# geduardo/SPARC

Measured on AMD Instinct MI355X. Metric: env-steps/sec at batch 65536, higher is better.
Workload: dtype f32 wire temperature + f64 scalar state

## Files before the change

### sparc_amd/csrc/wedm_common.h

```cpp
#pragma once


#ifndef WEDM_PACKED_DENSE
#define WEDM_PACKED_DENSE true
#endif
#ifndef WEDM_FUSED_DENSE
#define WEDM_FUSED_DENSE false
#endif
#ifndef WEDM_FUSED_MIN_BLOCKS
#define WEDM_FUSED_MIN_BLOCKS 2
#endif
#ifndef WEDM_PACKED_MIN_BLOCKS
#define WEDM_PACKED_MIN_BLOCKS 2
#endif
#ifndef WEDM_STREAM_PAIRED_LOADS
#define WEDM_STREAM_PAIRED_LOADS 1
#endif
#ifndef WEDM_STREAM_DENSE_QUIET
#define WEDM_STREAM_DENSE_QUIET 1
#endif
#ifndef WEDM_STREAM_REGWALK
#define WEDM_STREAM_REGWALK 1
#endif
#ifndef WEDM_PIN_STAGE
// ... 383 lines not shown
__device__ __forceinline__ void quad_f64(const f2 (&tm)[4], const f2 (&tc)[4], const f2 (&tp)[4], f2 (&tn)[4], const Geom& g,
                                         const f2 (&hc)[4], const Persist& ps, const f2 (&jfl)[4], const StencilF64& h, double jf64) {
    double cA = (double)hc[0].x * g.a64, cB = (double)hc[0].y * g.a64;
    double jA = (JOULE && jfl[0].x != 0.0f) ? jf64 : 0.0, jB = (JOULE && jfl[0].y != 0.0f) ? jf64 : 0.0;
#pragma unroll
    for (int u = 0; u < 4; ++u) {
        if (PERCELL && u > 0) {
            cA = (double)hc[u].x * g.a64; cB = (double)hc[u].y * g.a64;
            jA = (JOULE && jfl[u].x != 0.0f) ? jf64 : 0.0; jB = (JOULE && jfl[u].y != 0.0f) ? jf64 : 0.0;
        }
        tn[u].x = cell_f64<JOULE>(tm[u].x, tc[u].x, tp[u].x, g.k64, g.tuf64, cA, h.tdiel, ps.adv64, jA, h.alpha, h.tref);
#if WEDM_REGS_F64_FENCE < 0
        __builtin_amdgcn_sched_barrier(0);
#endif
        tn[u].y = cell_f64<JOULE>(tm[u].y, tc[u].y, tp[u].y, g.k64, g.tuf64, cB, h.tdiel, ps.adv64, jB, h.alpha, h.tref);
#if WEDM_REGS_F64_FENCE < 0
        __builtin_amdgcn_sched_barrier(0);
#elif WEDM_REGS_F64_FENCE > 0
        if ((u + 1) % WEDM_REGS_F64_FENCE == 0) __builtin_amdgcn_sched_barrier(0);
#endif
    }
}

template <bool F64, bool JOULE, bool PERCELL, int SW>
__device__ __forceinline__ void rw_quad(const f2 (&tm)[4], const f2 (&tc)[4], const f2 (&tp)[4], f2 (&tn)[4], const Geom& g,
                                        const f2 (&conv)[4], float tdiel, const Persist& ps, const f2 (&jfe)[4], float alpha,
                                        float tref, const StencilF64& h, const Coef& cf) {
    if (F64) quad_f64<JOULE, PERCELL>(tm, tc, tp, tn, g, conv, ps, jfe, h, cf.jf64);
    else quad_staged<JOULE, PERCELL, SW>(tm, tc, tp, tn, g.k, g.tuf, conv, tdiel, ps.adv, jfe, alpha, tref);
}
template <bool F64>
__device__ __forceinline__ float rw_cell(int i, int n_seg, float tm1, float tc, float tp1, const Geom& g, const Coef& cf,
                                         const Persist& ps, float tref, float alpha, float tdiel, const StencilF64& h,
                                         float h_base, float h_zone) {
    if (F64) return stencil_cell_f64(i, n_seg, tm1, tc, tp1, g, cf, ps, h, h_base, h_zone);
    return stencil_cell(i, n_seg, tm1, tc, tp1, g, cf, ps, tref, alpha, tdiel);
}

#define WEDM_REPORT_FROZEN(cond)                                                      \
    do {                                                                              \
        if (!kFrozenOk && __any(cond)) {                                              \
            int32_t* const seen = cold->frozen_seen;                                  \
            if (seen && (threadIdx.x & 63) == 0) *seen = 1;                           \
        }                                                                             \
    } while (0)

#ifdef WEDM_STAMPS
#define WEDM_STAMP(var)                                                      \
    do {                                                                     \
        __builtin_amdgcn_sched_barrier(0);                                   \
        asm volatile("s_memtime %0\n\ts_waitcnt lgkmcnt(0)" : "=s"(var)::"memory"); \
        __builtin_amdgcn_sched_barrier(0);                                   \
    } while (0)
#define WEDM_STAMP_DECL unsigned long long st0 = 0, st1 = 0, st2 = 0, st3 = 0, st4 = 0, acc0 = 0, acc1 = 0, acc2 = 0, acc3 = 0, tk0 = 0, tk1 = 0, accN = 0, accB = 0, accS = 0, cntN = 0, cntB = 0, cntS = 0
#define WEDM_STAMP_ACC() do { acc0 += st1 - st0; acc1 += st2 - st1; acc2 += st3 - st2; acc3 += st4 - st3; } while (0)
#define WEDM_STAMP_ACC_SPLIT(quiet)                                                             \
    do {                                                                                        \
        if (quiet) { WEDM_STAMP_ACC(); ++cntS; }                                                \
        else { accN += st1 - st0; accB += st2 - st1; accS += st4 - st2; ++cntN; }               \
    } while (0)
#define WEDM_STAMP_OUT()                                                                         \
    do {                                                                                         \
        if (k.dbg && (threadIdx.x & 63) == 0) {                                                  \
            unsigned long long* o = k.dbg + ((size_t)blockIdx.x * 4 + (threadIdx.x >> 6)) * 4;   \
            o[0] = acc0; o[1] = acc1; o[2] = acc2; o[3] = acc3;                                  \
            unsigned long long* o2 = k.dbg + (size_t)gridDim.x * 16 + ((size_t)blockIdx.x * 4 + (threadIdx.x >> 6)) * 6; \
            o2[0] = accN; o2[1] = accB; o2[2] = accS; o2[3] = cntN; o2[4] = cntB; o2[5] = cntS;  \
        }                                                                                        \
    } while (0)
#else
#define WEDM_STAMP(var) do { } while (0)
#define WEDM_STAMP_DECL do { } while (0)
#define WEDM_STAMP_ACC() do { } while (0)
#define WEDM_STAMP_ACC_SPLIT(quiet) do { } while (0)
#define WEDM_STAMP_OUT() do { } while (0)
#endif
```

### sparc_amd/csrc/wedm_device.h

```cpp
#pragma once

#include <hip/hip_runtime.h>
#include <stdint.h>

#include "../../include/wedm_hip.h"
#include "wedm_env_rows.h"

namespace wedm {

enum : uint32_t {
    F_TRACE = 1u << 0,
    F_F64 = 1u << 1,
    F_REPLAY = 1u << 2,
    F_PULSE = 1u << 3,
    F_ENVP = 1u << 4,
    F_MAT = 1u << 5,
    F_FROZEN_OK = 1u << 6,
    F_N1 = 1u << 7,
    F_EXTRA = 1u << 8,
    F_CUT = 1u << 9,
    F_ONE = 1u << 10,
    F_CMAX104 = 1u << 11,
    F_MINB2 = 1u << 12,
    F_SIG = 1u << 13,
// ... 92 lines not shown
struct W4 { uint32_t x, y, z, w; };

__device__ __forceinline__ W4 philox4(uint32_t key0, uint32_t key1, uint32_t time, uint32_t episode,
                                      uint32_t gid, uint32_t stream) {
    uint32_t c0 = time, c1 = episode, c2 = gid, c3 = stream, k0 = key0, k1 = key1;
#pragma unroll
    for (int r = 0; r < 10; ++r) {
        uint64_t p0 = (uint64_t)0xD2511F53u * c0;
        uint64_t p1 = (uint64_t)0xCD9E8D57u * c2;
        uint32_t n0 = (uint32_t)(p1 >> 32) ^ c1 ^ k0, n2 = (uint32_t)(p0 >> 32) ^ c3 ^ k1;
        c0 = n0; c1 = (uint32_t)p1; c2 = n2; c3 = (uint32_t)p0;
        k0 += 0x9E3779B9u;
        k1 += 0xBB67AE85u;
    }
    return W4{c0, c1, c2, c3};
}

__device__ __forceinline__ double u32_to_unit(uint32_t w) { return ((double)w + 0.5) * 2.3283064365386963e-10; }

struct U2 { double a, b; };
__device__ __forceinline__ U2 philox_pair(uint32_t key0, uint32_t key1, uint32_t time, uint32_t episode,
                                           uint32_t gid, uint32_t stream) {
    W4 w = philox4(key0, key1, time, episode, gid, stream);
    U2 u;
    u.a = ((double)(w.x >> 5) * 67108864.0 + (double)(w.y >> 6)) / 9007199254740992.0;
    u.b = ((double)(w.z >> 5) * 67108864.0 + (double)(w.w >> 6)) / 9007199254740992.0;
    return u;
}

__device__ __forceinline__ double philox_std_normal(uint32_t key0, uint32_t key1, uint32_t time,
                                                    uint32_t episode, uint32_t gid) {
    for (uint32_t j = 0; j < 64; ++j) {
        U2 u = philox_pair(key0, key1, time, episode, gid, 1u + j);
        double v1 = 2.0 * u.a - 1.0, v2 = 2.0 * u.b - 1.0;
        double s = v1 * v1 + v2 * v2;
        if (s < 1.0 && s != 0.0) return v1 * sqrt(-2.0 * portable_log(s) / s);
    }
    return 0.0;
}

struct Env {
    double wp, x, v, prev_a;
    double debris, rho, flow, last_gap, last_rho, wire_last_flow;
    double V, I, y, last_crater, cavity;
    double tdelta, tvolt, on, off, tpos, unwind;
    double ipk;
    double vacc;
    float h_base, h_zone, tmax;
    int32_t time, tss, tsov, tsi, tse, dur, rnd_rem, deb_rem, tcrit, mode, episode, sparks;
    uint32_t key0, key1;
    int32_t state;
    int32_t is_short, broken, reached, done, ctrl, err;
};

struct Hot {
    double hard_short_gap, base_critical_density, gap_coefficient, max_critical_density, sigmoid_steepness;
    double ignition_a, ignition_b, ignition_c, ln2;
    double default_target_voltage, default_on_time, default_off_time, spark_voltage_factor;
    double debris_removal_per_us;
    double dt_s, damping_coeff, stiffness_coeff, omega_n, max_acceleration, max_jerk_dt, max_speed;
    float spool, tref, alpha, tdiel, tcrit, tbreak;
    int32_t servo_interval, dt_us, control_mode, disable_ignition, has_random_short, per_env_geometry;
    uint32_t env_id_offset;
    int32_t n_seg;
    int32_t done_value;
};

__device__ __forceinline__ void pin_hot_in_vgprs(Hot& h) {
#define WEDM_PIN(x) asm volatile("" : "+v"(h.x))
    WEDM_PIN(hard_short_gap); WEDM_PIN(base_critical_density); WEDM_PIN(gap_coefficient);
    WEDM_PIN(max_critical_density); WEDM_PIN(sigmoid_steepness);
    WEDM_PIN(ignition_a); WEDM_PIN(ignition_b); WEDM_PIN(ignition_c); WEDM_PIN(ln2);
    WEDM_PIN(default_target_voltage); WEDM_PIN(default_on_time); WEDM_PIN(default_off_time);
    WEDM_PIN(spark_voltage_factor); WEDM_PIN(debris_removal_per_us);
    WEDM_PIN(dt_s); WEDM_PIN(damping_coeff); WEDM_PIN(stiffness_coeff); WEDM_PIN(omega_n);
    WEDM_PIN(max_acceleration); WEDM_PIN(max_jerk_dt); WEDM_PIN(max_speed);
#undef WEDM_PIN
}

__device__ __forceinline__ const double* kernarg_envp();
#define WEDM_ENVP_ROW(rows, row, stride) ((rows)[(int64_t)(row) * (stride) + e])

__device__ __forceinline__ void envp_apply(Hot& h, int64_t stride, int64_t e) {
    const double* const r = kernarg_envp();
    h.base_critical_density = WEDM_ENVP_ROW(r, WEDM_EP_BASE_CRITICAL_DENSITY, stride);
    h.gap_coefficient = WEDM_ENVP_ROW(r, WEDM_EP_GAP_COEFFICIENT, stride);
    h.max_critical_density = WEDM_ENVP_ROW(r, WEDM_EP_MAX_CRITICAL_DENSITY, stride);
    h.hard_short_gap = WEDM_ENVP_ROW(r, WEDM_EP_HARD_SHORT_GAP, stride);
    h.sigmoid_steepness = WEDM_ENVP_ROW(r, WEDM_EP_SIGMOID_STEEPNESS, stride);
    h.spark_voltage_factor = WEDM_ENVP_ROW(r, WEDM_EP_SPARK_VOLTAGE_FACTOR, stride);
    h.debris_removal_per_us = WEDM_ENVP_ROW(r, WEDM_EP_DEBRIS_REMOVAL_PER_US, stride);
    h.tdiel = (float)WEDM_ENVP_ROW(r, WEDM_EP_DIELECTRIC_TEMPERATURE, stride);
    h.damping_coeff = WEDM_ENVP_ROW(r, WEDM_EP_DAMPING_COEFF, stride);
    h.stiffness_coeff = WEDM_ENVP_ROW(r, WEDM_EP_STIFFNESS_COEFF, stride);
    h.omega_n = WEDM_ENVP_ROW(r, WEDM_EP_OMEGA_N, stride);
    h.max_acceleration = WEDM_ENVP_ROW(r, WEDM_EP_MAX_ACCELERATION, stride);
    h.max_jerk_dt = WEDM_ENVP_ROW(r, WEDM_EP_MAX_JERK_DT, stride);
    h.max_speed = WEDM_ENVP_ROW(r, WEDM_EP_MAX_SPEED, stride);
}

__device__ __forceinline__ const double* kernarg_wmat();
#define WEDM_WMAT_ROW(rows, row, stride) ((rows)[(int64_t)(row) * (stride) + e])

__device__ __forceinline__ void wmat_apply(Hot& h, int64_t stride, int64_t e) {
    const double* const r = kernarg_wmat();
    h.alpha = (float)WEDM_WMAT_ROW(r, WEDM_WM_ALPHA_RHO, stride);
// ... 582 lines not shown
        cf.jf = 0.0f;
        cf.jf64 = 0.0;
        if (cf.joule_on) {
            const double joule_geom = p.per_env_geometry ? cc0->g.f64[(int64_t)WEDM_G_JOULE_GEOM * cc0->s.stride + e] : jg_u;
            cf.jf64 = joule_geom * I2 * (MAT ? WEDM_WMAT_ROW(kernarg_wmat(), WEDM_WM_RHO_ELEC, cc0->s.stride) : rho_elec);
            cf.jf = (float)cf.jf64;
        }
    }
    return cf;
}

__device__ __forceinline__ bool pair_lane_b() { return (threadIdx.x & 1u) != 0u; }
__device__ __forceinline__ uint32_t pair_from_a(uint32_t x) { return (uint32_t)__builtin_amdgcn_mov_dpp((int32_t)x, 0xA0, 0xF, 0xF, true); }
__device__ __forceinline__ uint32_t pair_from_b(uint32_t x) { return (uint32_t)__builtin_amdgcn_mov_dpp((int32_t)x, 0xF5, 0xF, 0xF, true); }
__device__ __forceinline__ double pair_from_a(double x) {
    const uint64_t u = d2bits(x);
    return bits2d(((uint64_t)pair_from_a((uint32_t)(u >> 32)) << 32) | pair_from_a((uint32_t)u));
}
__device__ __forceinline__ double pair_from_b(double x) {
    const uint64_t u = d2bits(x);
    return bits2d(((uint64_t)pair_from_b((uint32_t)(u >> 32)) << 32) | pair_from_b((uint32_t)u));
}

#ifndef WEDM_PAIR_KEYS_HOISTED
#define WEDM_PAIR_KEYS_HOISTED 0
#endif
#ifndef WEDM_PAIR_DIV
#define WEDM_PAIR_DIV 1
#endif
struct PhiloxHalf { uint32_t X, lo; };
__device__ __forceinline__ PhiloxHalf philox4_pair(bool lane_b, uint32_t key0, uint32_t key1, uint32_t time, uint32_t episode,
                                                   uint32_t gid, uint32_t stream) {
#if !WEDM_PAIR_KEYS_HOISTED
    uint32_t odd = lane_b ? 1u : 0u;
    asm volatile("" : "+v"(odd));
    lane_b = odd != 0u;
#endif
    const uint32_t mul = lane_b ? 0xCD9E8D57u : 0xD2511F53u, weyl = lane_b ? 0xBB67AE85u : 0x9E3779B9u;
    uint32_t X = lane_b ? gid : time, lo = lane_b ? episode : stream, k = lane_b ? key1 : key0;
#pragma unroll
    for (int r = 0; r < 10; ++r) {
        const uint64_t m = (uint64_t)mul * X;
        const uint32_t t = (uint32_t)(m >> 32) ^ lo;
        lo = (uint32_t)m;
        X = (uint32_t)swap_with_neighbour((int32_t)t) ^ k;
        k += weyl;
    }
    return PhiloxHalf{X, lo};
}
__device__ __forceinline__ W4 philox4_pair_words(PhiloxHalf h) {
    return W4{pair_from_a(h.X), pair_from_b(h.lo), pair_from_b(h.X), pair_from_a(h.lo)};
}

template <bool DENSE, uint32_t F = 0, bool PAIR = false>
__device__ __forceinline__ bool quiet_prelude_t(const Hot& p, const ColdRef cold, const Geom& g, int64_t e, uint32_t gid,
                                                Env& s, QuietTry& qt, Coef& cf) {
    constexpr bool ENVP = (F & F_ENVP) != 0, MAT = (F & F_MAT) != 0;
    qt.have_w = false;
    if (p.disable_ignition || p.has_random_short) return false;
    const bool live = !s.done;
    const double d0 = s.wp - s.x;
    const bool idle = s.state == 0, rest = s.state == -2;
    const bool spk = DENSE && s.state == 1;
    double crit = p.base_critical_density + p.gap_coefficient * d0;
    crit = crit < p.max_critical_density ? crit : p.max_critical_density;
    const double ex = -p.sigmoid_steepness * (s.rho - crit);
    bool q = (s.tss < p.servo_interval) && (s.rnd_rem == 0) && (s.deb_rem == 0) && (idle || rest || spk) &&
             (d0 >= p.hard_short_gap) && (ex > 24.0);
    const double cavity = g.cavity_coeff * (d0 * 0.001);
    double rho = 0.0;
    double lam_pair = 0.0;
    if (PAIR && WEDM_PAIR_DIV) {
        const bool lane_b = pair_lane_b();
        const double den = p.ignition_a * (d0 * d0) + p.ignition_b * d0 + p.ignition_c;
        const double quot = (lane_b ? p.ln2 : s.debris) / (lane_b ? den : cavity);
        const double qq = pair_from_a(quot);
        lam_pair = pair_from_b(quot);
        if (cavity > 0) rho = qq < 1.0 ? qq : 1.0;
    } else if (cavity > 0) {
        const double qq = s.debris / cavity;
        rho = qq < 1.0 ? qq : 1.0;
    }
    q = q && !(__builtin_fabs(d0 - s.last_gap) > 0.01 || __builtin_fabs(rho - s.last_rho) > 0.001) &&
        !(__builtin_fabs(s.flow - s.wire_last_flow) > 0.01) && (d0 > 0.001);
    if (!__all(q || !live)) return false;
    bool ign = false;
    PhiloxHalf wh{0u, 0u};
    if (__any(idle && live)) {
        if (PAIR) {
            wh = philox4_pair(pair_lane_b(), s.key0, s.key1, (uint32_t)s.time, (uint32_t)s.episode, gid, 0u);
            if (!WEDM_PAIR_DIV) lam_pair = p.ln2 / (p.ignition_a * (d0 * d0) + p.ignition_b * d0 + p.ignition_c);
            ign = idle && live && (u32_to_unit(pair_from_b(wh.X)) < lam_pair);
        } else {
            const double lam = p.ln2 / (p.ignition_a * (d0 * d0) + p.ignition_b * d0 + p.ignition_c);
            const W4 w = philox4(s.key0, s.key1, (uint32_t)s.time, (uint32_t)s.episode, gid, 0u);
            ign = idle && live && (u32_to_unit(w.z) < lam);
#ifndef WEDM_NO_PHILOX_REUSE
            qt.w = w;
#endif
        }
#ifndef WEDM_NO_PHILOX_REUSE
        qt.have_w = true;
#endif
    }
    if (__any(ign)) {
#ifndef WEDM_NO_PHILOX_REUSE
        if (PAIR) qt.w = philox4_pair_words(wh);
#endif
        return false;
    }
    bool burning = false;
    if (live) {
        const double Vt = s.tvolt != 0.0 ? s.tvolt : p.default_target_voltage;
        const double on = s.on != 0.0 ? s.on : p.default_on_time;
        const double off = s.off != 0.0 ? s.off : p.default_off_time;
        const int32_t dur1 = s.dur + 1;
        const bool end_rest = rest && ((double)dur1 >= on + off);
        const bool end_on = spk && ((double)dur1 >= on);
        burning = spk && !end_on;
        s.ctrl = 0;
        s.is_short = 0;
        double V = idle ? Vt : (end_rest ? Vt : 0.0);
        if (DENSE) V = spk ? (end_on ? 0.0 : Vt * p.spark_voltage_factor) : V;
        s.V = V;
        s.I = burning ? s.ipk : 0.0;
        s.y = end_rest ? __builtin_nan("") : s.y;
        s.dur = idle ? s.dur : (end_rest ? 0 : dur1);
        s.state = end_rest ? 0 : (end_on ? -2 : s.state);
        s.last_crater = 0.0;
        s.cavity = cavity;
        s.rho = rho;
        if (s.flow > 0.001 && s.debris > 0.001) {
            const double nv = s.debris - p.debris_removal_per_us * s.flow;
            s.debris = nv > 0.0 ? nv : 0.0;
        }
    }
    if (DENSE && __any(burning)) {
        const ColdPtr cc0 = cold.get();
        const ParamsPtr c = opaque(cc0->p);
        const double seg = c->segment_len, eff = c->plasma_efficiency, rho_elec = c->rho_elec;
        const int zone_start = (p.per_env_geometry && burning) ? cc0->g.i32[(int64_t)WEDM_GI_ZONE_START * cc0->s.stride + e] : c->zone_start;
        const double joule_geom = (p.per_env_geometry && burning) ? cc0->g.f64[(int64_t)WEDM_G_JOULE_GEOM * cc0->s.stride + e] : c->joule_geom;
        if (burning && s.y == s.y) {
            const int idx = seg != 0 ? zone_start + spark_cell_offset(s.y, seg) : zone_start;
            if (idx >= 0 && idx < g.n_seg) {
                cf.pidx = idx;
                cf.q64 = (ENVP ? WEDM_ENVP_ROW(kernarg_envp(), WEDM_EP_PLASMA_EFFICIENCY, cc0->s.stride) : eff) * s.V * s.I;
                cf.q = (float)cf.q64;
            }
        }
        if (burning) {
            const double I2 = s.I * s.I;
            cf.joule_on = I2 > 1e-6;
            if (cf.joule_on) {
                cf.jf64 = joule_geom * I2 * (MAT ? WEDM_WMAT_ROW(kernarg_wmat(), WEDM_WM_RHO_ELEC, cc0->s.stride) : rho_elec);
                cf.jf = (float)cf.jf64;
            }
        }
    }
    return true;
}

__device__ __forceinline__ bool quiet_prelude(const Hot& p, const Geom& g, uint32_t gid, Env& s, QuietTry& qt) {
    Coef unused{0.0f, 0.0f, 0, -1};
    return quiet_prelude_t<false>(p, ColdRef{nullptr}, g, 0, gid, s, qt, unused);
}

__device__ __forceinline__ bool quiet_prelude(const Hot& p, const Geom& g, uint32_t gid, Env& s) {
    QuietTry qt;
    return quiet_prelude(p, g, gid, s, qt);
}

__device__ __forceinline__ float sub_twice(float a, float b) { return __builtin_fmaf(-2.0f, b, a); }
typedef float f2v __attribute__((ext_vector_type(2)));
__device__ __forceinline__ f2v sub_twice(f2v a, f2v b) {
    const f2v m2 = {-2.0f, -2.0f};
    return __builtin_elementwise_fma(m2, b, a);
}

__device__ __forceinline__ float stencil_cell(int i, int n_seg, float tm1, float tc, float tp1, const Geom& g,
                                              const Coef& c, const Persist& ps, float tref, float alpha,
                                              float tdiel) {
// ... 326 lines not shown
```

### sparc_amd/csrc/wedm_env_rows.h

```cpp
#pragma once

#define WEDM_ENV_F64_DOUBLES(X, a) \
    X(a, wp,             WEDM_F_WORKPIECE_POS,  PRE_GENERAL, IN,          STATE)  \
    X(a, x,              WEDM_F_WIRE_POS,       EPILOGUE,    IN,          STATE)  \
    X(a, v,              WEDM_F_WIRE_VEL,       EPILOGUE,    IN,          STATE)  \
    X(a, prev_a,         WEDM_F_PREV_ACCEL,     EPILOGUE,    IN,          MODULE) \
    X(a, debris,         WEDM_F_DEBRIS_VOLUME,  PRE_QUIET,   IN,          MODULE) \
    X(a, rho,            WEDM_F_DEBRIS_DENSITY, PRE_QUIET,   IN,          STATE)  \
    X(a, flow,           WEDM_F_FLOW,           PRE_GENERAL, IN,          MODULE) \
    X(a, last_gap,       WEDM_F_LAST_GAP,       PRE_GENERAL, IN,          MODULE) \
    X(a, last_rho,       WEDM_F_LAST_DENSITY,   PRE_GENERAL, IN,          MODULE) \
    X(a, wire_last_flow, WEDM_F_WIRE_LAST_FLOW, PRE_GENERAL, IN,          MODULE) \
    X(a, V,              WEDM_F_VOLTAGE,        PRE_QUIET,   IN,          STATE)  \
    X(a, I,              WEDM_F_CURRENT,        PRE_QUIET,   IN_FORCED,   STATE)  \
    X(a, y,              WEDM_F_SPARK_Y,        PRE_QUIET,   IN,          STATE)  \
    X(a, last_crater,    WEDM_F_LAST_CRATER,    PRE_QUIET,   OUT,         STATE)  \
    X(a, cavity,         WEDM_F_CAVITY,         PRE_QUIET,   OUT,         STATE)  \
    X(a, tdelta,         WEDM_F_TARGET_DELTA,   PRE_GENERAL, IN,          STATE)  \
    X(a, tvolt,          WEDM_F_TARGET_VOLTAGE, PRE_GENERAL, IN,          STATE)  \
    X(a, on,             WEDM_F_ON_TIME,        PRE_GENERAL, IN,          STATE)  \
    X(a, off,            WEDM_F_OFF_TIME,       PRE_GENERAL, IN,          STATE)  \
    X(a, tpos,           WEDM_F_TARGET_POS,     NEVER,       IN,          STATE)  \
    X(a, unwind,         WEDM_F_UNWIND_VEL,     NEVER,       IN,          STATE)
#define WEDM_ENV_F64_SUMS(X, a) \
    X(a, vacc,           WEDM_F_VOLT_ACC,       EPILOGUE,    IN,          STATE)
#define WEDM_ENV_F64_FLOATS(X, a) \
    X(a, h_base,         WEDM_F_H_BASE,         PRE_GENERAL, IN,          MODULE) \
    X(a, h_zone,         WEDM_F_H_ZONE,         PRE_GENERAL, IN,          MODULE) \
    X(a, tmax,           WEDM_F_TMAX,           EPILOGUE,    IN_KEEPSTEP, STATE)
#define WEDM_ENV_F64(X, a) WEDM_ENV_F64_DOUBLES(X, a) WEDM_ENV_F64_SUMS(X, a) WEDM_ENV_F64_FLOATS(X, a)

#define WEDM_ENV_I32(X, a) \
    X(a, time,           WEDM_I_TIME,             EPILOGUE,    IN,        STATE)  \
    X(a, tss,            WEDM_I_SINCE_SERVO,      EPILOGUE,    IN,        STATE)  \
    X(a, tsov,           WEDM_I_SINCE_OPEN_V,     EPILOGUE,    IN,        STATE)  \
    X(a, tsi,            WEDM_I_SINCE_IGNITION,   EPILOGUE,    IN,        STATE)  \
    X(a, tse,            WEDM_I_SINCE_SPARK_END,  EPILOGUE,    IN,        STATE)  \
    X(a, dur,            WEDM_I_SPARK_DUR,        PRE_QUIET,   IN,        STATE)  \
    X(a, rnd_rem,        WEDM_I_RANDOM_SHORT_REM, PRE_GENERAL, IN,        MODULE) \
    X(a, deb_rem,        WEDM_I_DEBRIS_SHORT_REM, PRE_GENERAL, IN,        MODULE) \
    X(a, tcrit,          WEDM_I_TIME_CRITICAL,    EPILOGUE,    IN,        STATE)  \
    X(a, mode,           WEDM_I_CURRENT_MODE,     PRE_GENERAL, IN,        STATE)  \
    X(a, episode,        WEDM_I_EPISODE,          NEVER,       IN,        STATE)  \
    X(a, key0,           WEDM_I_KEY_LO,           NEVER,       IN,        STATE)  \
    X(a, key1,           WEDM_I_KEY_HI,           NEVER,       IN,        STATE)  \
    X(a, sparks,         WEDM_I_SPARK_COUNT,      PRE_GENERAL, IN,        MODULE)

#define WEDM_ENV_I8(X, X_DONE, a) \
    X(a, state,          WEDM_B_SPARK_STATE,      PRE_QUIET,   IN,        STATE)  \
    X(a, is_short,       WEDM_B_IS_SHORT,         PRE_QUIET,   IN_FORCED, STATE)  \
    X(a, broken,         WEDM_B_WIRE_BROKEN,      EPILOGUE,    IN,        STATE)  \
    X(a, reached,        WEDM_B_TARGET_REACHED,   EPILOGUE,    IN,        STATE)  \
    X_DONE(a, done,      WEDM_B_DONE,             EPILOGUE,    IN,        STATE)  \
    X(a, ctrl,           WEDM_B_CTRL_STEP,        PRE_QUIET,   OUT,       STATE)  \
    X(a, err,            WEDM_B_ERROR,            PRE_GENERAL, IN,        STATE)

#define WEDM_UNHELD_F64(X) X(WEDM_F_VOLT_SUM, STATE, "VOLT_SUM is published at control steps only")
#define WEDM_UNHELD_I32(X) X(WEDM_I_TIME_HI, STATE, "TIME_HI is maintained at the end of a launch only")
#define WEDM_UNHELD_I8(X) X(WEDM_B_MODE_CACHED, MODULE, "MODE_CACHED is set in memory by the latching step")

namespace wedm {
enum : uint32_t {
    ROW_PRE_QUIET = 1u << 0, ROW_PRE_GENERAL = 1u << 1, ROW_EPILOGUE = 1u << 2, ROW_NEVER = 1u << 3,
    ROW_IN = 1u << 4, ROW_OUT = 1u << 5, ROW_IN_FORCED = 1u << 6, ROW_IN_KEEPSTEP = 1u << 7,
    ROW_STATE = 1u << 8, ROW_MODULE = 1u << 9,
    ROW_STORED = ROW_PRE_QUIET | ROW_PRE_GENERAL | ROW_EPILOGUE, ROW_ALL = ROW_IN | ROW_OUT | ROW_IN_FORCED | ROW_IN_KEEPSTEP,
};
#define WEDM_HAS(set, stage, role, owner) (((ROW_##stage | ROW_##role | ROW_##owner) & (set)) != 0)
#define WEDM_ROW_BIT(set, m, row, stage, role, owner) | (WEDM_HAS(set, stage, role, owner) ? 1u << (row) : 0u)
#define WEDM_F64_ROWS(set) (0u WEDM_ENV_F64(WEDM_ROW_BIT, set))
#define WEDM_I32_ROWS(set) (0u WEDM_ENV_I32(WEDM_ROW_BIT, set))
#define WEDM_I8_ROWS(set) (0u WEDM_ENV_I8(WEDM_ROW_BIT, WEDM_ROW_BIT, set))
#define WEDM_UNHELD_BIT(row, owner, why) | 1u << (row)
#define WEDM_UNHELD_MODULE_BIT(row, owner, why) | (ROW_##owner == ROW_MODULE ? 1u << (row) : 0u)

#define WEDM_CHECK_HOMES(B, count) \
    static_assert((WEDM_##B##_ROWS(ROW_ALL) | (0u WEDM_UNHELD_##B(WEDM_UNHELD_BIT))) == (1u << (count)) - 1u && \
                  (WEDM_##B##_ROWS(ROW_ALL) & (0u WEDM_UNHELD_##B(WEDM_UNHELD_BIT))) == 0, "every " #B " state row needs exactly one home: " \
                  "a line of WEDM_ENV_" #B " or an entry of WEDM_UNHELD_" #B " (wedm_env_rows.h)")
WEDM_CHECK_HOMES(F64, WEDM_F64_COUNT);
WEDM_CHECK_HOMES(I32, WEDM_I32_COUNT);
WEDM_CHECK_HOMES(I8, WEDM_I8_COUNT);
static_assert(WEDM_F64_ROWS(ROW_NEVER) == ((1u << WEDM_F_TARGET_POS) | (1u << WEDM_F_UNWIND_VEL)) && WEDM_I8_ROWS(ROW_NEVER) == 0 &&
              WEDM_I32_ROWS(ROW_NEVER) == ((1u << WEDM_I_EPISODE) | (1u << WEDM_I_KEY_LO) | (1u << WEDM_I_KEY_HI)),
              "stage NEVER is for the rows that no step assigns (target position, unwinding velocity, episode, RNG key): "
              "store_env() and the single-microsecond kernel's store_env_after_* would not persist any other row marked so");
}
```

### sparc_amd/csrc/wedm_k_regs.h

```cpp
#pragma once

struct cv4 {
    f2 v[4];
    __device__ __forceinline__ explicit cv4(f2 x) : v{x, x, x, x} {}
};

__device__ __forceinline__ float max3_raw(float a, float b, float c) {
    float r;
    asm("v_max3_f32 %0, %1, %2, %3" : "=v"(r) : "v"(a), "v"(b), "v"(c));
    return r;
}


#define WEDM_REGS_F64_CONSTS()                                                                                \
    StencilF64 f64c{0.0, 0.0, 0.0};                                                                           \
    if (F64) {                                                                                                \
        const wedm_params* pp = cold->p;                                                                      \
        f64c = StencilF64{pp->temp_ref, pp->alpha_rho, pp->dielectric_temperature};                           \
        g.k64 = pp->k_cond; g.tuf64 = pp->tuf; g.a64 = pp->a_surf;                                            \
    }
#define WEDM_REGS_LOAD_WIRE()                                                                                 \
    const int nq = (n + 3) >> 2;                                                                              \
    float* Te = cold->s.T + (live ? e : 0) * 4;                                                               \
    const int q0 = base / 4;                                                                                  \
    f2 P[H];                                                                                                  \
    _Pragma("unroll") for (int q = 0; q < H / 4; ++q) {                                                       \
        const f4v a = (q0 + q < nq) ? *(const f4v*)(Te + (int64_t)(q0 + q) * stride * 4) : f4v{0.0f, 0.0f, 0.0f, 0.0f}; \
        const f4v b = (q0 + H / 4 + q < nq) ? *(const f4v*)(Te + (int64_t)(q0 + H / 4 + q) * stride * 4) : f4v{0.0f, 0.0f, 0.0f, 0.0f}; \
        _Pragma("unroll") for (int u = 0; u < 4; ++u) P[4 * q + u] = f2{a[u], b[u]};                          \
    }
#define WEDM_REGS_WIPE_WIRE()                                                                                 \
    if (__any(reinit)) {                                                                                      \
        _Pragma("unroll") for (int m = 0; m < H; ++m) P[m] = reinit ? f2{spool, spool} : P[m];                \
    }                                                                                                         \
    if (c == 0) P[0].x = spool;
#define WEDM_REGS_STORE_WIRE()                                                                                \
    if (live) {                                                                                               \
        _Pragma("unroll") for (int q = 0; q < 2 * H / 4; ++q) {                                               \
            const int m = (q % (H / 4)) * 4;                                                                  \
            const bool hi = q >= H / 4;                                                                       \
            const f4v w = hi ? f4v{P[m].y, P[m + 1].y, P[m + 2].y, P[m + 3].y} : f4v{P[m].x, P[m + 1].x, P[m + 2].x, P[m + 3].x}; \
            const int cell = base + 4 * q;                                                                    \
            if (cell + 3 < n) {                                                                               \
                *(f4v*)(Te + (int64_t)(q0 + q) * stride * 4) = w;                                             \
            } else {                                                                                          \
                _Pragma("unroll") for (int u = 0; u < 4; ++u)                                                 \
                    if (cell + u < n) Te[(int64_t)(q0 + q) * stride * 4 + u] = w[u];                          \
            }                                                                                                 \
        }                                                                                                     \
    }

#ifndef WEDM_REGS_DENSE
#define WEDM_REGS_DENSE WEDM_PACKED_DENSE
#endif
#ifndef WEDM_REGS_SW2
#define WEDM_REGS_SW2 2
#endif
#ifndef WEDM_REGS_PIN2
#define WEDM_REGS_PIN2 1
#endif
#ifndef WEDM_REGS_PAIR_SPLIT
#define WEDM_REGS_PAIR_SPLIT 1
#endif
template <int L, uint32_t F>
__global__ void __launch_bounds__(256, L) wedm_step_regs(const KArgs k) {
    static_assert((F & ~(F_TRACE | F_F64 | F_PULSE)) == 0, "forms of wedm_step_regs");
    constexpr bool TRACE = (F & F_TRACE) != 0, F64 = (F & F_F64) != 0, PULSE = (F & F_PULSE) != 0;
    constexpr int CELLS = 128;
    constexpr int H = CELLS / (2 * L);
    static_assert(L == 1 || L == 2, "one or two lanes per environment");
    static_assert(H % 8 == 0 && H / 8 <= 16, "whole tiles");
    constexpr int EPB = 256 / L;
    constexpr int SW = L == 1 ? 4 : WEDM_REGS_SW2;
    constexpr bool kF64 = F64;
    const ColdRef cold = kernarg_cold();
    Hot hv = k.hot;
    if (L == 1 || WEDM_REGS_PIN2 == 2) {
        pin_hot_in_vgprs(hv);
    } else if (WEDM_REGS_PIN2 == 1) {
        pin_mechanics_in_vgprs(hv);
        pin_quiet_in_vgprs(hv);
    }
    const int tid = threadIdx.x;
    const int c = tid % L;
    int64_t e = (int64_t)blockIdx.x * EPB + tid / L;
    const uint32_t wave_env0 = __builtin_amdgcn_readfirstlane((uint32_t)e);
    auto env_index = [&]() -> int64_t {
        uint32_t all = ~0u;
        asm volatile("" : "+s"(all));
        const uint32_t lane = __builtin_amdgcn_mbcnt_hi(all, __builtin_amdgcn_mbcnt_lo(all, 0u));
        return (int64_t)(wave_env0 + lane / L);
    };
    const bool live = e < k.num_envs;
    const bool writer = c == 0;
    const WalkTable* __restrict__ wt = k.walk;
    const int n = k.hot.n_seg;
    const int64_t stride = cold->s.stride;
    const int base = c * 2 * H;

    Env s;
    Geom g;
    Persist ps{0.0f, 0.0f, 0.0f, 0};
    load_geom(k.hot, cold, live ? e : 0, g);
    WEDM_REGS_F64_CONSTS()
    WEDM_ENV_LOAD()
    WEDM_REGS_LOAD_WIRE()
    const float spool = k.hot.spool, tref = k.hot.tref, alpha = k.hot.alpha, tdiel = k.hot.tdiel;
    Sig none;
    WEDM_ENV_RESET(writer, none, )
    WEDM_REGS_WIPE_WIRE()
    WEDM_ENV_START(const bool frozen0, )

    static_assert(H / 8 <= 8, "tile flags: a byte per mask");
    const int n_tiles = wt->n_tiles;
    uint32_t tile_flags = 0u, joule_any = 0u;
    for (int t = 0; t < n_tiles; ++t) {
        const uint32_t lo = wt->zj[8 * t];
        tile_flags |= (((lo >> (2 * c)) & 1u) << t) | (((lo >> (2 * c + 1)) & 1u) << (8 + t));
        tile_flags |= (((lo >> (16 + 2 * c)) & 1u) << (16 + t)) | (((lo >> (17 + 2 * c)) & 1u) << (24 + t));
        joule_any |= ((lo >> 16) != 0u ? 1u : 0u) << t;
    }
    if (L == 1) tile_flags = __builtin_amdgcn_readfirstlane(tile_flags);
    joule_any = __builtin_amdgcn_readfirstlane(joule_any);
    const uint32_t kind_n = __builtin_amdgcn_readfirstlane(wt->kind_n_mask);
    const uint32_t kind_ne = __builtin_amdgcn_readfirstlane(wt->kind_ne_mask), kind_nj = __builtin_amdgcn_readfirstlane(wt->kind_nj_mask);
    const int last_base = (2 * L - 1) * H;
    const uint32_t last_tile = (n > last_base) ? (1u << ((n - 1 - last_base) >> 3)) : 0u;
    const bool owns_last = c == L - 1;

    f2 convp[H / 8];
    auto build_conv = [&]() {
        const uint32_t zoneA = tile_flags & 0xFFu, zoneB = (tile_flags >> 8) & 0xFFu;
        const float cz = F64 ? s.h_zone : ps.conv_zone, cb = F64 ? s.h_base : ps.conv_base;
#pragma unroll
        for (int t = 0; t < H / 8; ++t)
            convp[t] = f2{((zoneA >> t) & 1u) ? cz : cb, ((zoneB >> t) & 1u) ? cz : cb};
    };
    build_conv();
    WEDM_STAMP_DECL;
    const bool tracing = WEDM_TRACING(k);
    int trace_next = k.trace_next, trace_slot = k.trace_slot;
    (void)trace_next; (void)trace_slot;

    for (int it = 0; it < k.n_substeps; ++it) {
        if (__all(s.done) && !tracing) break;
        WEDM_STAMP(st0);
        e = env_index();
        const uint32_t gid = k.hot.env_id_offset + (uint32_t)e;
        const int32_t pk = PULSE ? pulse_kind(s) : 0;
        Coef cf{0.0f, 0.0f, 0, -1};
        QuietTry qt;
        const bool was_quiet = quiet_prelude_t<WEDM_REGS_DENSE, 0u, L == 2 && WEDM_REGS_PAIR_SPLIT>(hv, cold, g, e, gid, s, qt, cf);
        if (!was_quiet) {
            if (!s.done) cf = scalar_prelude(hv, cold, g, e, gid, s, ps, writer, qt);
            build_conv();
        }
        freeze_wire(s);
        WEDM_STAMP(st1);
        const bool act = !s.done;
        float tmax = spool;
        if (L == 1) asm volatile("" : "+s"(tile_flags));
        else asm volatile("" : "+v"(tile_flags));
        const uint32_t jouleA = (tile_flags >> 16) & 0xFFu, jouleB = tile_flags >> 24;
        Geom gw = g;
        gw.n_seg = __builtin_amdgcn_readfirstlane(g.n_seg); gw.az_start = __builtin_amdgcn_readfirstlane(g.az_start);
        gw.az_end = __builtin_amdgcn_readfirstlane(g.az_end); gw.cb = __builtin_amdgcn_readfirstlane(g.cb);
        gw.ct = __builtin_amdgcn_readfirstlane(g.ct);
        asm volatile("" : "+s"(gw.n_seg), "+s"(gw.az_start), "+s"(gw.az_end), "+s"(gw.cb), "+s"(gw.ct));
        int nw = __builtin_amdgcn_readfirstlane(n);
        asm volatile("" : "+s"(nw));
        const float a_last = P[H - 1].x, b_first = P[0].y;
        float halo_l = spool, halo_r = 0.0f;
        if (L == 2) {
            const float give = c == 0 ? P[H - 1].y : P[0].x;
            const float got = __int_as_float(swap_with_neighbour(__float_as_int(give)));
            halo_l = c == 0 ? spool : got;
            halo_r = c == 0 ? got : 0.0f;
        }
        const float rw_h_base = s.h_base, rw_h_zone = s.h_zone;
#include "wedm_regs_walk.inc"
        WEDM_STAMP(st2);
        if (L == 2) tmax = fmax_gt(tmax, __int_as_float(swap_with_neighbour(__float_as_int(tmax))));
        WEDM_ENV_END_US(hv, tmax, pk, writer, none, WEDM_STAMP(st3))
        WEDM_STAMP(st4);
        WEDM_STAMP_ACC_SPLIT(was_quiet);
        WEDM_TRACE_POINT(k, it, e, s, writer,
                         float* pa = tT + (int64_t)base * tcnt; float* pb = pa + (int64_t)H * tcnt;
                         int na = n - base; int nb = na - H;
                         asm volatile("" : "+v"(na), "+v"(nb));
                         _Pragma("unroll") for (int m = 0; m < H; ++m) {
                             if (m < na) *pa = P[m].x;
                             if (m < nb) *pb = P[m].y;
                             pa += tcnt; pb += tcnt;
                             asm volatile("" : "+v"(pa), "+v"(pb));
                         });
    }
    WEDM_STAMP_OUT();

    e = env_index();
    Te = cold->s.T + (live ? e : 0) * 4;
    WEDM_REGS_STORE_WIRE()
    if (live && writer) { WEDM_ENV_CLOSE(frozen0) }
}


__device__ __forceinline__ float dpp_row_shr1(float old, float x) {
    return __int_as_float(__builtin_amdgcn_update_dpp(__float_as_int(old), __float_as_int(x), 0x111, 0xF, 0xF, false));
}
__device__ __forceinline__ float dpp_row_shl1(float old, float x) {
    return __int_as_float(__builtin_amdgcn_update_dpp(__float_as_int(old), __float_as_int(x), 0x101, 0xF, 0xF, false));
}
template <int CTRL>
__device__ __forceinline__ float dpp_perm(float x) {
    return __int_as_float(__builtin_amdgcn_update_dpp(0, __float_as_int(x), CTRL, 0xF, 0xF, false));
}

#ifndef WEDM_WIDE_MIN_BLOCKS
#define WEDM_WIDE_MIN_BLOCKS 1
#endif

#ifndef WEDM_WIDE_SW
#define WEDM_WIDE_SW 2
#endif
#ifndef WEDM_WIDE_DENSE
#define WEDM_WIDE_DENSE WEDM_REGS_DENSE
#endif
#ifndef WEDM_WIDE_AUTO_MAX_LANES
#define WEDM_WIDE_AUTO_MAX_LANES 65536
#endif
constexpr int wide_min_blocks(uint32_t F) { return !(F & F_F64) ? WEDM_WIDE_MIN_BLOCKS : (F & F_MINB2) ? 2 : 1; }
template <int L, uint32_t F>
__global__ void __launch_bounds__(256, wide_min_blocks(F)) wedm_step_regs_wide(const KArgs k) {
    static_assert((F & ~(F_CUT | F_TRACE | F_F64 | F_MINB2 | F_PULSE)) == 0 && (!(F & F_MINB2) || (F & F_F64)),
                  "forms of wedm_step_regs_wide");
    constexpr bool CUT = (F & F_CUT) != 0, TRACE = (F & F_TRACE) != 0, F64 = (F & F_F64) != 0, PULSE = (F & F_PULSE) != 0;
    constexpr int H = 16, MINB = wide_min_blocks(F);
    static_assert(H % 8 == 0 && H <= 32, "whole tiles");
    static_assert(L == 4 || L == 8 || L == 16, "the lanes of an environment lie in one DPP row");
    constexpr int EPB = 256 / L;
    constexpr int SW = WEDM_WIDE_SW;
    const ColdRef cold = kernarg_cold();
    Hot hv = k.hot;
    if (MINB == 1) pin_hot_in_vgprs(hv);
    const int tid = threadIdx.x;
    const int c = tid % L;
    const int64_t e = (int64_t)blockIdx.x * EPB + tid / L;
    const bool live = e < k.num_envs;
    const bool writer = c == 0;
    const int n = k.hot.n_seg;
    const int64_t stride = cold->s.stride;
    const int base = c * 2 * H;
// ... 215 lines not shown
```

### sparc_amd/csrc/wedm_lifecycle.h

```cpp
#pragma once

template <uint32_t F>
__device__ __forceinline__ Hot launch_hot(const KArgs& k, const ColdRef cold, int64_t e, bool live) {
    Hot hv = k.hot;
    if (F & (F_ENVP | F_MAT)) {
        const int64_t er = live ? e : 0;
        if (F & F_ENVP) envp_apply(hv, cold->s.stride, er);
        if (F & F_MAT) wmat_apply(hv, cold->s.stride, er);
    }
    return hv;
}

#define WEDM_ENV_LOAD()                                                                                       \
    if (live) load_env(cold, e, s);                                                                           \
    else { s.done = WEDM_DEAD_LANE; s.unwind = 0.0; s.h_base = 0.0f; s.h_zone = 0.0f; }

#define WEDM_ENV_RESET_UNDER(reinit, writer, sg, wipe)                                                        \
    if (reinit) {                                                                                             \
        reinit_env(cold, e, s, writer);                                                                       \
        pulse_reinit<(F & F_PULSE) != 0>(kernarg_pulse(), cold, e, writer);                                   \
        if constexpr ((F & F_SIG) != 0) sig_reinit<true>(kernarg_sig(), cold, e, writer, sg);                 \
        wipe;                                                                                                 \
    }
#define WEDM_ENV_RESET(writer, sg, wipe)                                                                      \
    const bool reinit = live && s.done && WEDM_AUTORESET(cold);                                               \
    WEDM_ENV_RESET_UNDER(reinit, writer, sg, wipe)

#define WEDM_ENV_START(frozen0, report)                                                                       \
    unfreeze_wire(k.hot, s);                                                                                  \
    frozen0 = s.done;                                                                                         \
    report;                                                                                                   \
    if (!s.done) {                                                                                            \
        s.ipk = peak_current(cold, s.mode, e);                                                                \
        init_persist<false, (F & F_MAT) != 0>(k.hot, cold, e, s, ps);                                         \
    }

#define WEDM_ENV_STEP_DONE(hv, tmax, prev_pulse, writer, sg)                                                  \
    scalar_epilogue(hv, s, tmax);                                                                             \
    pulse_tally<(F & F_PULSE) != 0>(kernarg_pulse(), cold, e, s, prev_pulse, writer);                         \
    if constexpr ((F & F_SIG) != 0) sig_tally<true, (F & F_PULSE) != 0>(kernarg_sig(), cold, e, s, writer, sg); \
    if (s.ctrl) control_step_outputs(cold, e, s, writer);
#define WEDM_ENV_END_US(hv, tmax, prev_pulse, writer, sg, mark)                                               \
    unfreeze_wire(hv, s);                                                                                     \
    mark;                                                                                                     \
    if (!s.done) { WEDM_ENV_STEP_DONE(hv, tmax, prev_pulse, writer, sg) }

#define WEDM_ENV_CLOSE(frozen0)                                                                               \
    if (WEDM_REWARD_ON(cold)) {                                                                               \
        if (!frozen0) write_reward(cold, e, s);                                                               \
        else cold->s.reward[e] = 0.0f;                                                                        \
    }                                                                                                         \
    store_time_hi(cold, e, s, (uint32_t)k.n_substeps * (uint32_t)k.hot.dt_us);                                \
    store_env(cold, e, s);

template <uint32_t F>
__device__ __forceinline__ bool env_open(const ColdRef cold, int64_t e, bool live, bool writer, Env& s) {
    WEDM_ENV_LOAD()
    Sig none;
    WEDM_ENV_RESET(writer, none, )
    return reinit;
}
template <uint32_t F>
__device__ __forceinline__ bool env_start(const KArgs& k, const ColdRef cold, int64_t e, Env& s, Persist& ps) {
    WEDM_ENV_START(const bool frozen0, )
    return frozen0;
}

template <uint32_t F>
__device__ __forceinline__ void env_step_done(const Hot& hv, const ColdRef cold, int64_t e, Env& s, float tmax, int32_t prev_pulse,
                                              bool writer, Sig& sg) {
    WEDM_ENV_STEP_DONE(hv, tmax, prev_pulse, writer, sg)
}
template <uint32_t F>
__device__ __forceinline__ void env_step_done(const Hot& hv, const ColdRef cold, int64_t e, Env& s, float tmax, int32_t prev_pulse,
                                              bool writer) {
    static_assert(!(F & F_SIG), "an F_SIG form hands in its accumulators");
    Sig none;
    env_step_done<F>(hv, cold, e, s, tmax, prev_pulse, writer, none);
}

template <uint32_t F>
__device__ __forceinline__ void env_end_us(const Hot& hv, const ColdRef cold, int64_t e, Env& s, float tmax, int32_t prev_pulse,
                                           bool writer, Sig& sg) {
    WEDM_ENV_END_US(hv, tmax, prev_pulse, writer, sg, )
}
template <uint32_t F>
__device__ __forceinline__ void env_end_us(const Hot& hv, const ColdRef cold, int64_t e, Env& s, float tmax, int32_t prev_pulse,
                                           bool writer) {
    static_assert(!(F & F_SIG), "an F_SIG form hands in its accumulators");
    Sig none;
    env_end_us<F>(hv, cold, e, s, tmax, prev_pulse, writer, none);
}

__device__ __forceinline__ void env_close(const KArgs& k, const ColdRef cold, int64_t e, const Env& s, bool frozen0, bool store) {
    if (!store) return;
    WEDM_ENV_CLOSE(frozen0)
}

// ... 9 lines not shown
```

Before: 16.83 billion.

## Park rarely-used env state fields in LDS to relieve VGPR pressure

Moves a set of cold or rarely touched Env members (mode, sparks, err, unwind, episode, h_base, h_zone, ctrl, is_short, last_crater) out of registers into a per-lane shared-memory slot array in the L==2 register kernel. Members are restored only on the non-quiet path and around the epilogue, and the quiet path zeroes parked fields in place. The aim is fewer live VGPRs, which allows higher occupancy or less spilling. The cost is extra LDS traffic, shared memory per block, and more complex state handling. It also adds a drained timing stamp for profiling builds.

```diff
diff --git a/sparc_amd/csrc/wedm_common.h b/sparc_amd/csrc/wedm_common.h
--- a/sparc_amd/csrc/wedm_common.h
+++ b/sparc_amd/csrc/wedm_common.h
@@ -459,11 +459,17 @@
         asm volatile("s_memtime %0\n\ts_waitcnt lgkmcnt(0)" : "=s"(var)::"memory"); \
         __builtin_amdgcn_sched_barrier(0);                                   \
     } while (0)
-#define WEDM_STAMP_DECL unsigned long long st0 = 0, st1 = 0, st2 = 0, st3 = 0, st4 = 0, acc0 = 0, acc1 = 0, acc2 = 0, acc3 = 0, tk0 = 0, tk1 = 0, accN = 0, accB = 0, accS = 0, cntN = 0, cntB = 0, cntS = 0
+#define WEDM_STAMP_DRAIN(var)                                                \
+    do {                                                                     \
+        __builtin_amdgcn_sched_barrier(0);                                   \
+        asm volatile("s_waitcnt vmcnt(0)\n\ts_memtime %0\n\ts_waitcnt lgkmcnt(0)" : "=s"(var)::"memory"); \
+        __builtin_amdgcn_sched_barrier(0);                                   \
+    } while (0)
+#define WEDM_STAMP_DECL unsigned long long st1w = 0, st0 = 0, st1 = 0, st2 = 0, st3 = 0, st4 = 0, acc0 = 0, acc1 = 0, acc2 = 0, acc3 = 0, tk0 = 0, tk1 = 0, accN = 0, accB = 0, accS = 0, cntN = 0, cntB = 0, cntS = 0
 #define WEDM_STAMP_ACC() do { acc0 += st1 - st0; acc1 += st2 - st1; acc2 += st3 - st2; acc3 += st4 - st3; } while (0)
 #define WEDM_STAMP_ACC_SPLIT(quiet)                                                             \
     do {                                                                                        \
-        if (quiet) { WEDM_STAMP_ACC(); ++cntS; }                                                \
+        if (quiet) { WEDM_STAMP_ACC(); ++cntS; cntB += st1w - st1; }                            \
         else { accN += st1 - st0; accB += st2 - st1; accS += st4 - st2; ++cntN; }               \
     } while (0)
 #define WEDM_STAMP_OUT()                                                                         \
@@ -477,6 +483,7 @@
     } while (0)
 #else
 #define WEDM_STAMP(var) do { } while (0)
+#define WEDM_STAMP_DRAIN(var) do { } while (0)
 #define WEDM_STAMP_DECL do { } while (0)
 #define WEDM_STAMP_ACC() do { } while (0)
 #define WEDM_STAMP_ACC_SPLIT(quiet) do { } while (0)
diff --git a/sparc_amd/csrc/wedm_device.h b/sparc_amd/csrc/wedm_device.h
--- a/sparc_amd/csrc/wedm_device.h
+++ b/sparc_amd/csrc/wedm_device.h
@@ -168,6 +168,32 @@
     int32_t state;
     int32_t is_short, broken, reached, done, ctrl, err;
 };
+
+struct ParkSlots {
+#define WEDM_PARK_SLOT(a, m, quiet) uint32_t m[sizeof(Env::m) / 4];
+    WEDM_ENV_PARKED(WEDM_PARK_SLOT, )
+#undef WEDM_PARK_SLOT
+};
+constexpr int PARK_ROWS = sizeof(ParkSlots) / 4;
+#define WEDM_PARK_ROW(m) ((int)(offsetof(wedm::ParkSlots, m) / 4))
+#define WEDM_PARK_BIT(m) (1u << WEDM_PARK_ROW(m))
+#define WEDM_PARK_IN_SET(a, m, quiet) | WEDM_PARK_BIT(m)
+constexpr uint32_t PARK_ALL = 0u WEDM_ENV_PARKED(WEDM_PARK_IN_SET, );
+#undef WEDM_PARK_IN_SET
+
+template <typename T>
+__device__ __forceinline__ void park_put(uint32_t (*slots)[256], int row, int lane, T v) {
+    static_assert(sizeof(T) == 4 || sizeof(T) == 8, "a parked member is one dword or two");
+    uint32_t w[sizeof(T) / 4];
+    __builtin_memcpy(w, &v, sizeof(T));
+    for (int i = 0; i < (int)(sizeof(T) / 4); ++i) slots[row + i][lane] = w[i];
+}
+template <typename T>
+__device__ __forceinline__ void park_get(uint32_t (*slots)[256], int row, int lane, T& v) {
+    uint32_t w[sizeof(T) / 4];
+    for (int i = 0; i < (int)(sizeof(T) / 4); ++i) w[i] = slots[row + i][lane];
+    __builtin_memcpy(&v, w, sizeof(T));
+}
 
 struct Hot {
     double hard_short_gap, base_critical_density, gap_coefficient, max_critical_density, sigmoid_steepness;
@@ -856,9 +882,9 @@
     return W4{pair_from_a(h.X), pair_from_b(h.lo), pair_from_b(h.X), pair_from_a(h.lo)};
 }
 
-template <bool DENSE, uint32_t F = 0, bool PAIR = false>
+template <bool DENSE, uint32_t F = 0, bool PAIR = false, uint32_t PARKED = 0>
 __device__ __forceinline__ bool quiet_prelude_t(const Hot& p, const ColdRef cold, const Geom& g, int64_t e, uint32_t gid,
-                                                Env& s, QuietTry& qt, Coef& cf) {
+                                                Env& s, QuietTry& qt, Coef& cf, uint32_t (*slots)[256] = nullptr, int lane = 0) {
     constexpr bool ENVP = (F & F_ENVP) != 0, MAT = (F & F_MAT) != 0;
     qt.have_w = false;
     if (p.disable_ignition || p.has_random_short) return false;
@@ -922,8 +948,11 @@
         const bool end_rest = rest && ((double)dur1 >= on + off);
         const bool end_on = spk && ((double)dur1 >= on);
         burning = spk && !end_on;
-        s.ctrl = 0;
-        s.is_short = 0;
+#define WEDM_QUIET_ZERO(m)                                                                   \
+    if constexpr ((PARKED & WEDM_PARK_BIT(m)) != 0) park_put(slots, WEDM_PARK_ROW(m), lane, decltype(Env::m)(0)); \
+    else s.m = 0
+        WEDM_QUIET_ZERO(ctrl);
+        WEDM_QUIET_ZERO(is_short);
         double V = idle ? Vt : (end_rest ? Vt : 0.0);
         if (DENSE) V = spk ? (end_on ? 0.0 : Vt * p.spark_voltage_factor) : V;
         s.V = V;
@@ -931,7 +960,8 @@
         s.y = end_rest ? __builtin_nan("") : s.y;
         s.dur = idle ? s.dur : (end_rest ? 0 : dur1);
         s.state = end_rest ? 0 : (end_on ? -2 : s.state);
-        s.last_crater = 0.0;
+        WEDM_QUIET_ZERO(last_crater);
+#undef WEDM_QUIET_ZERO
         s.cavity = cavity;
         s.rho = rho;
         if (s.flow > 0.001 && s.debris > 0.001) {
diff --git a/sparc_amd/csrc/wedm_env_rows.h b/sparc_amd/csrc/wedm_env_rows.h
--- a/sparc_amd/csrc/wedm_env_rows.h
+++ b/sparc_amd/csrc/wedm_env_rows.h
@@ -59,6 +59,18 @@
 #define WEDM_UNHELD_I32(X) X(WEDM_I_TIME_HI, STATE, "TIME_HI is maintained at the end of a launch only")
 #define WEDM_UNHELD_I8(X) X(WEDM_B_MODE_CACHED, MODULE, "MODE_CACHED is set in memory by the latching step")
 
+#define WEDM_ENV_PARKED(X, a) \
+    X(a, mode,        COLD) \
+    X(a, sparks,      COLD) \
+    X(a, err,         COLD) \
+    X(a, unwind,      COLD) \
+    X(a, episode,     READ) \
+    X(a, h_base,      COLD) \
+    X(a, h_zone,      COLD) \
+    X(a, ctrl,        ZERO) \
+    X(a, is_short,    ZERO) \
+    X(a, last_crater, ZERO)
+
 namespace wedm {
 enum : uint32_t {
     ROW_PRE_QUIET = 1u << 0, ROW_PRE_GENERAL = 1u << 1, ROW_EPILOGUE = 1u << 2, ROW_NEVER = 1u << 3,
diff --git a/sparc_amd/csrc/wedm_k_regs.h b/sparc_amd/csrc/wedm_k_regs.h
--- a/sparc_amd/csrc/wedm_k_regs.h
+++ b/sparc_amd/csrc/wedm_k_regs.h
@@ -59,6 +59,9 @@
 #ifndef WEDM_REGS_PIN2
 #define WEDM_REGS_PIN2 1
 #endif
+#ifndef WEDM_REGS_PARK
+#define WEDM_REGS_PARK 1
+#endif
 #ifndef WEDM_REGS_PAIR_SPLIT
 #define WEDM_REGS_PAIR_SPLIT 1
 #endif
@@ -73,6 +76,8 @@
     constexpr int EPB = 256 / L;
     constexpr int SW = L == 1 ? 4 : WEDM_REGS_SW2;
     constexpr bool kF64 = F64;
+    constexpr bool PARK = L == 2 && F == 0 && WEDM_REGS_PARK;
+    constexpr uint32_t PK = PARK ? PARK_ALL : 0u;
     const ColdRef cold = kernarg_cold();
     Hot hv = k.hot;
     if (L == 1 || WEDM_REGS_PIN2 == 2) {
@@ -91,6 +96,7 @@
         const uint32_t lane = __builtin_amdgcn_mbcnt_hi(all, __builtin_amdgcn_mbcnt_lo(all, 0u));
         return (int64_t)(wave_env0 + lane / L);
     };
+    auto park_lane = [&]() -> int { return tid; };
     const bool live = e < k.num_envs;
     const bool writer = c == 0;
     const WalkTable* __restrict__ wt = k.walk;
@@ -141,22 +147,31 @@
     const bool tracing = WEDM_TRACING(k);
     int trace_next = k.trace_next, trace_slot = k.trace_slot;
     (void)trace_next; (void)trace_slot;
+    if constexpr (PARK) env_park(park_slots(), park_lane(), s);
 
     for (int it = 0; it < k.n_substeps; ++it) {
         if (__all(s.done) && !tracing) break;
         WEDM_STAMP(st0);
+        if constexpr (PARK) env_unpark_read(park_slots(), park_lane(), s);
         e = env_index();
         const uint32_t gid = k.hot.env_id_offset + (uint32_t)e;
         const int32_t pk = PULSE ? pulse_kind(s) : 0;
         Coef cf{0.0f, 0.0f, 0, -1};
         QuietTry qt;
-        const bool was_quiet = quiet_prelude_t<WEDM_REGS_DENSE, 0u, L == 2 && WEDM_REGS_PAIR_SPLIT>(hv, cold, g, e, gid, s, qt, cf);
+        const bool was_quiet = quiet_prelude_t<WEDM_REGS_DENSE, 0u, L == 2 && WEDM_REGS_PAIR_SPLIT, PK>(hv, cold, g, e, gid, s, qt, cf, PARK ? park_slots() : nullptr, PARK ? park_lane() : 0);
+        int32_t ctrl_now = 0;
         if (!was_quiet) {
+            if constexpr (PARK) env_unpark(park_slots(), park_lane(), s);
             if (!s.done) cf = scalar_prelude(hv, cold, g, e, gid, s, ps, writer, qt);
             build_conv();
+            if constexpr (PARK) {
+                ctrl_now = s.ctrl;
+                env_park(park_slots(), park_lane(), s);
+            }
         }
         freeze_wire(s);
         WEDM_STAMP(st1);
+        WEDM_STAMP_DRAIN(st1w);
         const bool act = !s.done;
         float tmax = spool;
         if (L == 1) asm volatile("" : "+s"(tile_flags));
@@ -177,11 +192,11 @@
             halo_l = c == 0 ? spool : got;
             halo_r = c == 0 ? got : 0.0f;
         }
-        const float rw_h_base = s.h_base, rw_h_zone = s.h_zone;
+        const float rw_h_base = PARK ? 0.0f : s.h_base, rw_h_zone = PARK ? 0.0f : s.h_zone;
 #include "wedm_regs_walk.inc"
         WEDM_STAMP(st2);
         if (L == 2) tmax = fmax_gt(tmax, __int_as_float(swap_with_neighbour(__float_as_int(tmax))));
-        WEDM_ENV_END_US(hv, tmax, pk, writer, none, WEDM_STAMP(st3))
+        WEDM_ENV_END_US_ON(hv, tmax, pk, writer, none, WEDM_STAMP(st3), (PK & WEDM_PARK_BIT(ctrl)) ? ctrl_now : s.ctrl)
         WEDM_STAMP(st4);
         WEDM_STAMP_ACC_SPLIT(was_quiet);
         WEDM_TRACE_POINT(k, it, e, s, writer,
@@ -197,6 +212,7 @@
     }
     WEDM_STAMP_OUT();
 
+    if constexpr (PARK) env_unpark(park_slots(), park_lane(), s);
     e = env_index();
     Te = cold->s.T + (live ? e : 0) * 4;
     WEDM_REGS_STORE_WIRE()
diff --git a/sparc_amd/csrc/wedm_lifecycle.h b/sparc_amd/csrc/wedm_lifecycle.h
--- a/sparc_amd/csrc/wedm_lifecycle.h
+++ b/sparc_amd/csrc/wedm_lifecycle.h
@@ -44,6 +44,42 @@
     unfreeze_wire(hv, s);                                                                                     \
     mark;                                                                                                     \
     if (!s.done) { WEDM_ENV_STEP_DONE(hv, tmax, prev_pulse, writer, sg) }
+
+#define WEDM_ENV_STEP_DONE_ON(hv, tmax, prev_pulse, writer, sg, ctrl_step)                                    \
+    scalar_epilogue(hv, s, tmax);                                                                             \
+    pulse_tally<(F & F_PULSE) != 0>(kernarg_pulse(), cold, e, s, prev_pulse, writer);                         \
+    if constexpr ((F & F_SIG) != 0) sig_tally<true, (F & F_PULSE) != 0>(kernarg_sig(), cold, e, s, writer, sg); \
+    if (ctrl_step) control_step_outputs(cold, e, s, writer);
+#define WEDM_ENV_END_US_ON(hv, tmax, prev_pulse, writer, sg, mark, ctrl_step)                                 \
+    unfreeze_wire(hv, s);                                                                                     \
+    mark;                                                                                                     \
+    if (!s.done) { WEDM_ENV_STEP_DONE_ON(hv, tmax, prev_pulse, writer, sg, ctrl_step) }
+
+__device__ __forceinline__ void env_park(uint32_t (*slots)[256], int lane, const Env& s) {
+#define WEDM_PARK_PUT(a, m, quiet) park_put(slots, WEDM_PARK_ROW(m), lane, s.m);
+    WEDM_ENV_PARKED(WEDM_PARK_PUT, )
+#undef WEDM_PARK_PUT
+}
+__device__ __forceinline__ void env_unpark(uint32_t (*slots)[256], int lane, Env& s) {
+#define WEDM_PARK_GET(a, m, quiet) park_get(slots, WEDM_PARK_ROW(m), lane, s.m);
+    WEDM_ENV_PARKED(WEDM_PARK_GET, )
+#undef WEDM_PARK_GET
+}
+__device__ __forceinline__ void env_unpark_read(uint32_t (*slots)[256], int lane, Env& s) {
+#define WEDM_PARK_GET_COLD(m)
+#define WEDM_PARK_GET_ZERO(m)
+#define WEDM_PARK_GET_READ(m) park_get(slots, WEDM_PARK_ROW(m), lane, s.m);
+#define WEDM_PARK_GET(a, m, quiet) WEDM_PARK_GET_##quiet(m)
+    WEDM_ENV_PARKED(WEDM_PARK_GET, )
+#undef WEDM_PARK_GET
+#undef WEDM_PARK_GET_READ
+#undef WEDM_PARK_GET_ZERO
+#undef WEDM_PARK_GET_COLD
+}
+__device__ __forceinline__ uint32_t (*park_slots())[256] {
+    __shared__ uint32_t slots[PARK_ROWS][256];
+    return slots;
+}
 
 #define WEDM_ENV_CLOSE(frozen0)                                                                               \
     if (WEDM_REWARD_ON(cold)) {                                                                               \
```

Measured after the change: 16.93 billion, median of 6. Within noise of the previous version (+0.6%).
